# jackvial/tuatara

Measured on AMD Instinct MI355X. Metric: pages/sec whole-node (1024x768, ~40 crops/page), higher is better.
Workload: dtype f16x4

## Files before the change

### tuatara_amd/csrc/capi_debug.cpp

```cpp
#include "engine.h"

using namespace ttr;

extern "C" {

int ttr_dbg_conv(ttr_engine* e, const float* in0, int C0, const float* in1, int C1, int relu0, int relu1, int B, int H, int W, int ks, int dil,
                 const float* wgt, const float* bias, int Cout, int act, float* out) {
  TTR_GUARD_BEGIN
  Engine& E = *e->e;
  EngineScope lk(E);
  const size_t M = (size_t)B * H * W;
  const int K = ks * ks * (C0 + C1);
  DevBuf d0, d1, dout;
  Linear L;
  auto up = [&](DevBuf& d, const float* src, size_t nel) {
    d.ensure(nel * E.es);
    if (E.prec == kBF16) {
      std::vector<uint16_t> hbuf(nel);
      for (size_t i = 0; i < nel; ++i) hbuf[i] = f32_to_bf16_rne(src[i]);
      TTR_HIP_CHECK(hipMemcpy(d.p, hbuf.data(), nel * 2, hipMemcpyHostToDevice));
    } else TTR_HIP_CHECK(hipMemcpy(d.p, src, nel * 4, hipMemcpyHostToDevice));
  };
  up(d0, in0, M * C0);
  if (C1) up(d1, in1, M * C1);
// ... 308 lines not shown

void ttr_set_gemm_config(int cfg) { set_gemm_config(cfg); }

void ttr_set_decoder_mode(int mode) { g_tuning_default.decoder_mode = mode; }

void ttr_last_host_us(ttr_engine* e, float out[8]) { for (int i = 0; i < 8; ++i) out[i] = e ? e->e->host_us[i] : 0.f; }

int ttr_dbg_dec_stamps_ext(unsigned long long* out, int n) { return g_dec_dbg && n >= 0 && n <= 4096 && hipMemcpy(out, g_dec_dbg, (size_t)n * 8, hipMemcpyDeviceToHost) == hipSuccess ? 0 : -1; }
int ttr_dbg_dec_stamps(unsigned long long* out) { return g_dec_dbg && hipMemcpy(out, g_dec_dbg, 26 * 16 * 8, hipMemcpyDeviceToHost) == hipSuccess ? 0 : -1; }

int ttr_set_tuning(const char* key, int value) {
  const std::string k = key ? key : "";
  if (g_tuning_default.set(k, value)) return 0;
  if (k == "gemm_config") set_gemm_config(value);
  else if (k == "self_refine") set_dec_self_refine(value);
  else if (k == "cross_mfma") set_dec_cross_mfma(value);
  else if (k == "cross_crop") set_dec_cross_crop(value);
  else if (k == "cross_split") set_dec_cross_split(value);
  else if (k == "cross_rows_hsplit") set_dec_cross_rows_hsplit(value);
  else if (k == "mlp_store_nt") set_mlp_store_nt(value);
  else if (k == "mlp_stagger") set_mlp_stagger(value);
  else if (k == "c3s_wgs") set_conv3s_wgs_per_cu(value);
  else if (k == "c3_c32") set_conv3p_c32_tile(value);
  else if (k == "c3_narrow64") set_conv3p_narrow_bn64(value);
  else if (k == "upsample_block") set_upsample_block(value);
  else if (k == "mlp_ablate") set_mlp_ablate(value);
  else if (k == "attn_impl") set_attn_impl(value);
  else if (k == "ws_dbg_flags") set_gemm_ws_dbg_flags(value);
  else if (k == "ws_lean") set_gemm_ws_lean(value);
  else if (k == "store_policy") set_store_policy(value);
  else if (k == "head_persistent") set_conv3p_head_persistent(value);
  else if (k == "up_resident") set_gemm2_up_resident(value);
  else if (k == "up_2d") set_gemm2_up_2d(value);
  else if (k == "c3h_wgs_per_cu") set_conv3h_wgs_per_cu(value);
  else if (k == "g2_x_ring3") set_gemm2_x_ring3(value);
  else if (k == "g2_split_reuse") set_gemm2_split_reuse(value);
  else if (k == "g2_split_cfg") set_gemm2_split_cfg(value);
  else if (k == "g2_split_few") set_gemm2_split_few(value);
  else if (k == "g2_split_dbg") set_gemm2_split_dbg(value);
  else if (k == "g2_split_wreg") set_gemm2_split_wreg(value);
  else if (k == "g2_split_stream") set_gemm2_split_stream(value);
  else if (k == "g2_split_stream4") set_gemm2_split_stream4(value);
  else if (k == "gsp_sched") set_gemm_sp_sched(value);
  else if (k == "gsp_few") set_gemm_sp_few(value);
  else if (k == "gsp_epi") set_gemm_sp_epi(value);
  else if (k == "gsp_ks3") set_gemm_sp_ks3(value);
  else if (k == "gsp_stagger") set_gemm_sp_stagger(value);
  else if (k == "gsp_dbg") set_gemm_sp_dbg(value);
  else if (k == "gsp_stag") set_gemm_sp_stag(value);
  else if (k == "gsp_stagger_groups") set_gemm_sp_stagger_groups(value);
  else if (k == "qkv_attn_dbg") set_qkv_attn_dbg(value);
  else if (k == "qkv_attn4") set_qkv_attn4(value);
  else if (k == "skx_ln_max_rows") set_gemm_skx_ln_max_rows(value);
  else if (k == "c3_xs1_max_cin") set_conv3p_single_stage_max_cin(value);
  else if (k == "c3_force_bn128") set_conv3p_force_bn128(value);
  else if (k == "c3_c64_waves") set_conv3p_c64_waves(value);
  else if (k == "c3_c128_waves") set_conv3p_c128_waves(value);
  else if (k == "c3_narrow_wide") set_conv3p_narrow_wide(value);
  else if (k == "c3_narrow_frac") set_conv3p_narrow_frac(value);
  else if (k == "c3_narrowest_frac") set_conv3p_narrowest_frac(value);
  else if (k == "c3_deep_w") set_conv3p_deep_w(value);
  else if (k == "c3_deep_w64") set_conv3p_deep_w64(value);
  else if (k == "c3_first_persistent") set_conv3p_first_persistent(value);
  else if (k == "sk_max_rows") set_skinny_max_rows(value);
  else if (k == "ws_min_rows") set_gemm_ws_min_rows(value);
  else if (k == "dec_stamps") {
    if (value && !g_dec_dbg) { void* d = nullptr; if (hipMalloc(&d, 4096 * 8) != hipSuccess) return -1; (void)hipMemset(d, 0, 4096 * 8); g_dec_dbg = (unsigned long long*)d; }
    if (!value) g_dec_dbg = nullptr;
    set_gemm_ws_stamps(value == 2 ? g_dec_dbg : nullptr);
    set_conv3p_stamps(value == 4 ? g_dec_dbg : nullptr);
    set_mlp_stamps(value == 3 ? g_dec_dbg : nullptr);
    set_qkv_attn_stamps(value == 5 ? g_dec_dbg : nullptr);
    set_qkv_attn4_stamps(value == 5 ? g_dec_dbg : nullptr);
    set_conv3h_stamps(value == 6 ? g_dec_dbg : nullptr);
  }
  else return -1;
  return 0;
}

int ttr_engine_set_tuning(ttr_engine* e, const char* key, int value) {
  TTR_GUARD_BEGIN
  if (!e) return -1;
  const std::string k = key ? key : "";
  {
    std::lock_guard<std::mutex> lk(e->e->mu);
    if (e->e->tn.set(k, value)) return 0;
  }
  return ttr_set_tuning(key, value);
  TTR_GUARD_END(-1)
}

int ttr_bench_conv(ttr_engine* e, int B, int H, int W, int C0, int C1, int ks, int dil, int Cout, int act, int f32_resid, int iters, float* avg_us) {
  TTR_GUARD_BEGIN
  Engine& E = *e->e;
  EngineScope lk(E);
  const size_t M = (size_t)B * H * W;
  const int K = ks * ks * (C0 + C1);
  DevBuf d0, d1, dw, db, dout, dres;
  d0.ensure(M * C0 * E.es); launch_fill_random(E.prec, d0.p, M * C0, 1u, 1.0f, E.stream);
  if (C1) { d1.ensure(M * C1 * E.es); launch_fill_random(E.prec, d1.p, M * C1, 2u, 1.0f, E.stream); }
  dw.ensure((size_t)Cout * K * E.es); launch_fill_random(E.prec, dw.p, (size_t)Cout * K, 3u, 1.0f / std::sqrt((float)K), E.stream);
  db.ensure((size_t)Cout * 4); launch_fill_random(kF32, db.p, Cout, 4u, 1.0f, E.stream);
  ConvParams p{};
  p.in0 = d0.p; p.C0 = C0; p.in1 = C1 ? d1.p : nullptr; p.C1 = C1;
  p.B = B; p.H = H; p.W = W; p.ks = ks; p.dil = dil; p.wgt = dw.p; p.bias = db.as<float>();
  p.Cout = Cout; p.M = (int)M; p.act = act;
// ... 95 lines not shown
```

### tuatara_amd/csrc/engine.h

```cpp
#pragma once
#include <algorithm>
#include <cmath>
#include <cstdio>
#include <cstring>
#include <fstream>
#include <iostream>
#include <iterator>
#include <map>
#include <memory>
#include <mutex>
#include <chrono>
#include <dlfcn.h>
#include <arpa/inet.h>
#include <netdb.h>
#include <netinet/in.h>
#include <netinet/tcp.h>
#include <sys/socket.h>
#include <unistd.h>
#include <rccl/rccl.h>

#include <atomic>
#include <functional>
#include <condition_variable>
#include <thread>
#include <stdexcept>
#include <string>
#include <vector>

#include "../../include/tuatara_hip_debug.h"
#include "common.h"
#include "geometry.h"
#include "host_util.h"
#include "kernels.h"

namespace ttr {


extern thread_local std::string g_last_error;
extern unsigned long long* g_dec_dbg;
struct Tuning {
  int dbg_bf16_out = 0;
  int qkv_attn = 1;
  int qkv_attn_min = 160;
  int mlp_proj = 1;
  int mlp_min_rows = 49152;
  int dec_mlp_fused = 1;
  int dec_mlp_min_rows = 16384;
  int mlp_fused = 1;
  int tok_fuse = 1;
  int ln_fuse = 1;
  int fuse_first = 1;
  int qkv_attn_split = 1;
  int skinny_split = 1;
  int skinny_max_rows = 2048;
  int skx_ln_fuse = 1;
  int embed_fold = 1;
  int argmax_fold = 1;
  int sp_tiled_x = 1;
  int sp_tiled_w = 1;
  int ar_host_check = 10;
  int enc_chunk = 0;
  int enc_ln_pairs = 1;
  int dec_planes = 1;
  int qkv_kv_pairs = 1;
  int enc_fc2_pairs = 1;
  int craft_products = 3;
  int gpu_calipers = 1;
  int up_commute = 1;
  int head_tail = 1;
  int first_fused = 1;
  int head_packed = 1;
  int detector_only = 0;
  int bench_grid_boxes = 0;
  int split_planes = 1;
  int split_conv3p = 1;
  int split_gemm = 1;
  int craft_group = 16;
  int ar_tail_step = 12;
  int ar_crop_exit = 1;
  int ar_early_exit = 1;
  int decoder_mode = 1;
  int sp_hidden16 = 0;
  int craft_lanes = 1;
  int recog_overlap = 1;
  int images_batch = 32;
  int range_guard = 1;
  bool set(const std::string& k, int value) {
    if (k == "decoder_mode") decoder_mode = value;
    else if (k == "enc_chunk") enc_chunk = value;
    else if (k == "range_guard") range_guard = value;
    else if (k == "recog_overlap") recog_overlap = value;
    else if (k == "craft_lanes") craft_lanes = value == 2 ? 2 : 1;
    else if (k == "sp_hidden16") sp_hidden16 = value;
    else if (k == "images_batch") images_batch = value < 1 ? 1 : (value > 256 ? 256 : value);
    else if (k == "up_commute") up_commute = value;
    else if (k == "gpu_calipers") gpu_calipers = value;
    else if (k == "skinny_split") skinny_split = value;
    else if (k == "skinny_max_rows") skinny_max_rows = value;
    else if (k == "ar_host_check") ar_host_check = value;
    else if (k == "sp_tiled_w") sp_tiled_w = value;
    else if (k == "sp_tiled_x") sp_tiled_x = value;
    else if (k == "argmax_fold") argmax_fold = value;
    else if (k == "embed_fold") embed_fold = value;
    else if (k == "skx_ln_fuse") skx_ln_fuse = value;
    else if (k == "qkv_attn_split") qkv_attn_split = value;
    else if (k == "fuse_first") fuse_first = value;
    else if (k == "ln_fuse") ln_fuse = value;
// ... 560 lines not shown
```

### tuatara_amd/csrc/engine_parseq.cpp

```cpp
#include "engine.h"

namespace ttr {

unsigned long long* g_dec_dbg = nullptr;

void Engine::sgemm(const Linear& L, const void* in_planes, int M, void* out, int out_ld, int act, int out_planes,
           float* out_f32, int out_f32_ld, const float* resid, int resid_ld, int np, int resid_mod, int out_full_cols,
           const char* kind, int x_tiled, int out_tiled) {
  if (!L.ws.p) throw std::runtime_error("split GEMM: the layer has no weight planes");
  range_tag("parseq." + range_scope + (kind ? kind : "linear"));
  ConvParams p{};
  p.out_full_cols = out_full_cols;
  p.in0 = in_planes; p.C0 = L.k; p.B = 1; p.H = 1; p.W = M; p.ks = 1; p.dil = 1;
  p.wgt = L.ws.p; p.bias = L.b.as<float>(); p.split = np; p.out_scale = L.inv_scale; p.out_planes = out_planes == 1 ? 3 : out_planes;
  p.wgt_tiled = tn.sp_tiled_w ? L.wst.p : nullptr;
  p.x_tiled = x_tiled; p.out_tiled = out_tiled;
  p.store_policy = out_tiled == 2 && tn.sp_hidden16 == 2 ? 1 : 0;
  p.out = out; p.out_ld = out_ld; p.out_f32 = out_f32; p.out_f32_ld = out_f32_ld; p.resid = resid; p.resid_ld = resid_ld; p.resid_mod = resid_mod;
  p.Cout = L.cout_valid ? L.cout_valid : L.cout; p.M = M; p.act = act;
  p.skip = cur_skip; p.skip_n = cur_skip_n;
  const bool skinny = tn.skinny_split && np == 4 && M <= tn.skinny_max_rows && !x_tiled && !out_tiled && gemm_skx_eligible(p);
  if (!skinny) { if (const char* e = gemm2_check(p)) throw std::runtime_error(e); }
  if (skinny) {
    timed(kind ? kind : "split linear (triples, skinny)", 2.0 * M * p.Cout * L.k, 2.0 * M * p.Cout * L.k * np, [&] { launch_gemm_skx(p, stream); });
// ... 53 lines not shown
    p.Cout = L.cout_valid ? L.cout_valid : L.cout; p.M = rows; p.act = act;
    p.skip = cur_skip; p.skip_n = cur_skip_n;
    if (tn.skx_ln_fuse && tn.skinny_split && L.ws.p && gemm_skx_ln_eligible(p)) {
      timed(kind, 2.0 * rows * p.Cout * L.k, 2.0 * rows * p.Cout * L.k * 4, [&] { launch_gemm_skx(p, stream); });
      return;
    }
    lnp(nm, pa);
    sgemm(L, pa, rows, out, out_ld, act, out_planes, out_f32, out_f32_ld, nullptr, 0, 4, 0, 0, kind);
  };
  range_tag("parseq.decoder.self_attn.out_proj");
  sgemm(pq.at("self_out"), sa, rows, nullptr, 0, kActNone, 0, tgt, 384, resid_pos, 384, 4, resid_mod);
  ln_lin(d + "norm1", pq.at("cross_q"), q384, 384, kActNone, 0, nullptr, 0, "dec.norm1 + cross_q");
  range_tag("parseq.decoder.cross_attn");
  launch_dec_cross_attn(kF32, q384, kvmem, pb, N, R, stream, cur_skip, cur_skip_n, done_tok, done_col, 3);
  sgemm(pq.at("cross_out"), pb, rows, nullptr, 0, kActNone, 0, tgt, 384, tgt, 384);
  ln_lin(d + "norm2", pq.at("ffn1"), p1536, 1536, kActGelu, 3, nullptr, 0, "dec.norm2 + ffn1");
  sgemm(pq.at("ffn2"), p1536, rows, nullptr, 0, kActNone, 0, tgt, 384, tgt, 384);
  const Linear& head = pq.at("head");
  if (head.ws.p && tn.skinny_split && rows <= tn.skinny_max_rows)
    ln_lin("decoder.norm", head, nullptr, 0, kActNone, 0, logits_out, logits_ld, "dec.norm + head (skinny)");
  else ln_gemm(tgt, "decoder.norm", 1e-5f, t384, head, rows, nullptr, 0, kActNone, logits_out, logits_ld);
}

void Engine::decoder_tail(const void* sa, int N, int R, const float* resid_pos, int resid_mod, float* tgt, void* t384, void* t384b, void* t1536,
                  const void* kvmem, float* logits_out, int logits_ld, const int* done_tok, int done_col) {
  const int rows = N * R;
  const std::string d = "decoder.layers.0.";
  gemm(pq.at("self_out"), sa, rows, nullptr, 0, kActNone, tgt, 384, resid_pos, 384, resid_mod);
  ln_gemm(tgt, d + "norm1", 1e-5f, t384, pq.at("cross_q"), rows, t384b, 384, kActNone);
  launch_dec_cross_attn(prec, t384b, kvmem, t384, N, R, stream, cur_skip, cur_skip_n, done_tok, done_col);
  const int dec_panels = (rows + 127) / 128, dec_cus = device_cu_count(256), dec_rounds = (dec_panels + dec_cus - 1) / dec_cus;
  const bool dec_fill = tn.dec_mlp_fused == 2 || dec_panels * 100 >= 65 * dec_rounds * dec_cus;
  if (R > 1 && prec == kBF16 && gemm_config() >= 0 && tn.dec_mlp_fused && rows >= tn.dec_mlp_min_rows && dec_fill) {
    MlpParams q{};
    q.x = tgt; q.x_out = tgt; q.M = rows;
    q.ln_g = pqf.at(d + "norm2.weight").as<float>(); q.ln_b = pqf.at(d + "norm2.bias").as<float>(); q.ln_eps = 1e-5f;
    q.w1p = dec_ffn1_packed.as<bf16>(); q.b1 = pq.at("ffn1").b.as<float>();
    q.w2p = dec_ffn2_packed.as<bf16>(); q.b2 = pq.at("ffn2").b.as<float>();
    q.nln_g = pqf.at("decoder.norm.weight").as<float>(); q.nln_b = pqf.at("decoder.norm.bias").as<float>(); q.nln_eps = 1e-5f; q.nln_out = (bf16*)t384b;
    q.att = (const bf16*)t384; q.wpp = dec_co_packed.as<bf16>(); q.bp = pq.at("cross_out").b.as<float>();
    timed("mlp_fused (refinement block)", 2.0 * rows * 384 * 1536 * 2 + 2.0 * rows * 384 * 384, 2.0 * rows * 384 * 1536 * 2 + 2.0 * rows * 384 * 384, [&] { launch_mlp_fused(q, stream); });
    gemm(pq.at("head"), t384b, rows, nullptr, 0, kActNone, logits_out, logits_ld);
    return;
  }
  gemm(pq.at("cross_out"), t384, rows, nullptr, 0, kActNone, tgt, 384, tgt, 384, 0);
  ln_gemm(tgt, d + "norm2", 1e-5f, t384, pq.at("ffn1"), rows, t1536, 1536, kActGelu);
  gemm(pq.at("ffn2"), t1536, rows, nullptr, 0, kActNone, tgt, 384, tgt, 384, 0);
  ln_gemm(tgt, "decoder.norm", 1e-5f, t384, pq.at("head"), rows, nullptr, 0, kActNone, logits_out, logits_ld);
}

void Engine::parseq_forward(const uint8_t* d_crops, int N, float* d_logits, float* d_ar, int* d_ids, float* d_prob, float* d_conf, const RowMask* row_masks,
                            int* d_alt_ids, float* d_alt_prob) {
  if (N <= 0) return;
  constexpr int kMaxCrops = 4096;
  if (N > kMaxCrops) {
    const int groups = (N + kMaxCrops - 1) / kMaxCrops, per = (N + groups - 1) / groups;
    for (int g0 = 0; g0 < N; g0 += per) {
      const int n = std::min(per, N - g0);
      parseq_forward(d_crops + (size_t)g0 * 32 * 128 * 3, n, d_logits + (size_t)g0 * 26 * 95, d_ar ? d_ar + (size_t)g0 * 26 * 95 : nullptr, d_ids + (size_t)g0 * 26,
                     d_prob + (size_t)g0 * 26, d_conf + g0, row_masks ? row_masks + g0 : nullptr,
                     d_alt_ids ? d_alt_ids + (size_t)g0 * 26 * alts : nullptr, d_alt_prob ? d_alt_prob + (size_t)g0 * 26 * alts : nullptr);
    }
    return;
  }
  if ((charset.restricts() || row_masks) && prec == kBF16) throw std::runtime_error("parseq_forward: a character set needs an f16x4 or f32 engine (the bf16 engine's kernels take no class mask)");
  prof_stage = 1;
  const int M = N * 128, E = 384;
  const int patch_ld = pq.at("patch").k;
  range_tag("parseq.encoder.patch_embed");
  void* patches = (pq_ws[0].ensure((size_t)M * patch_ld * es), pq_ws[0].p);
  float* x = (float*)(pq_ws[1].ensure((size_t)M * E * 4), pq_ws[1].p);
  void* t384 = (pq_ws[2].ensure((size_t)std::max(M, N * 26) * E * es), pq_ws[2].p);
  void* tbig = (pq_ws[3].ensure((size_t)M * 1536 * es), pq_ws[3].p);
  void* att = (pq_ws[4].ensure((size_t)std::max(M, N * 26) * E * es), pq_ws[4].p);
  launch_patchify(prec, d_crops, patches, N, patch_ld, stream);
  gemm(pq.at("patch"), patches, M, nullptr, 0, kActNone, x, E, pqf.at("encoder.pos_embed").as<float>(), E, 128);
  const bool enc_split = prec == kSplit && tn.split_gemm && tn.split_planes;
  if (enc_split) {
    int CHS = std::max(1, std::min(N, (int)((((size_t)1 << 31) - 1) / ((size_t)128 * 1536 * 6))));
    if (tn.enc_chunk > 0) CHS = std::min(CHS, tn.enc_chunk);
    if (N > CHS) { const int groups = (N + CHS - 1) / CHS; CHS = (N + groups - 1) / groups; }
    void* lnp = (pq_ws[11].ensure((size_t)M * E * 6), pq_ws[11].p);
    void* bigp = (pq_ws[12].ensure((size_t)std::min(N, CHS) * 128 * 1536 * 6), pq_ws[12].p);
    void* attp = (pq_ws[13].ensure((size_t)std::min(N, CHS) * 128 * E * 6), pq_ws[13].p);
    auto lnp_at = [&](int c0) { return (char*)lnp + (size_t)c0 * 128 * E * 6; };
    const int lnpl = tn.enc_ln_pairs ? 2 : 3;
    const int xt = tn.sp_tiled_x && tn.qkv_attn_split && lnpl == 2 && tn.enc_fc2_pairs && std::min(CHS, N) * 128 > tn.skinny_max_rows ? 1 : 0;
    for (int c0 = 0; c0 < N; c0 += CHS) {
      const int nc = std::min(CHS, N - c0), Mc = nc * 128;
      float* xc = x + (size_t)c0 * 128 * E;
      for (int l = 0; l < 12; ++l) {
        const std::string p = "encoder.blocks." + std::to_string(l) + ".";
        range_scope = p;
        range_tag("parseq." + p + "norm1");
        launch_layernorm_planes(xc, E, pqf.at(p + "norm1.weight").as<float>(), pqf.at(p + "norm1.bias").as<float>(), 1e-6f, lnp_at(c0), Mc, stream, lnpl, nullptr, 0, xt);
        if (tn.qkv_attn_split && lnpl == 2) {
          const Linear& L = pq.at(p + "qkv_hm");
          range_tag("parseq." + p + "attn (qkv + attention)");
          const double qa = 2.0 * Mc * 3 * E * E, aa = 2.0 * 2 * nc * 6 * 128.0 * 128 * 64;
          timed("enc.qkv+attention: gemm_sp_kernel<128,192,NP=3,EPI=1>", qa + aa, qa * 3 + aa * 3.5,
                [&] { launch_qkv_attn_split(lnp_at(c0), L.ws.p, L.b.as<float>(), L.inv_scale, attp, nc, stream, tn.sp_tiled_w ? L.wst.p : nullptr, xt, xt); });
        } else {
        sgemm(pq.at(p + "qkv"), lnp_at(c0), Mc, bigp, 3 * E, kActNone, 1, nullptr, 0, nullptr, 0, lnpl + 1, 0, tn.qkv_kv_pairs ? E : 0, "enc.qkv");
        range_tag("parseq." + p + "attn.qkv"), launch_attn_enc_split(bigp, attp, nc, stream);
        }
        sgemm(pq.at(p + "proj"), attp, Mc, nullptr, 0, kActNone, 0, xc, E, xc, E, 4, 0, 0, "enc.proj", xt, 0);
        range_tag("parseq." + p + "norm2");
// ... 209 lines not shown
```

### tuatara_amd/csrc/gemm_skx.hip

```cpp
#include <stdexcept>

#include "common.h"
#include "kernels.h"
#include "split.h"

namespace ttr {

namespace {
__device__ __forceinline__ __amdgpu_buffer_rsrc_t skx_rsrc(const void* base, unsigned bytes) {
  return __builtin_amdgcn_make_buffer_rsrc(const_cast<void*>(base), 0, (int)bytes, 0x00020000);
}
__device__ __forceinline__ f16x8 skx_load(__amdgpu_buffer_rsrc_t rs, unsigned voff, unsigned soff) {
  return __builtin_bit_cast(f16x8, __builtin_amdgcn_raw_buffer_load_b128(rs, voff, soff, 0));
}
constexpr int SKX_BN = 32, SKX_DEPTH = 3;
}

template <int RB, bool LNP = false, bool ROWM = false>
__global__ __launch_bounds__(256) void gemm_skx_kernel(ConvParams p) {
  static_assert(!LNP || RB == 1, "the LayerNorm prologue is the 16-row form's");
  static_assert(!ROWM || LNP, "row masks belong to the token prologue");
  __shared__ __attribute__((aligned(16))) float part[4][2][RB][64][4];
  __shared__ int skip_now;
  if (p.skip) {
    if (LNP && p.done_count) {
      if (threadIdx.x == 0) skip_now = __builtin_nontemporal_load(p.skip) >= p.skip_n;
      __syncthreads();
      if (skip_now) return;
    } else if (__builtin_nontemporal_load(p.skip) >= p.skip_n) return;
  }
  constexpr int XROW = 3 * 384 + 8;
  __shared__ __attribute__((aligned(16))) f16 xs[LNP ? 16 * XROW : 8];
  const int tid = threadIdx.x, lane = tid & 63;
  const int wave = __builtin_amdgcn_readfirstlane(tid >> 6);
  const int q = lane & 15, g = lane >> 4;
  RangeWatch rw;
  const int K = p.C0, nsteps = K >> 5;
  const int n0 = blockIdx.x * SKX_BN, m0 = blockIdx.y * (16 * RB);
  const __amdgpu_buffer_rsrc_t rsx = skx_rsrc(p.in0, (unsigned)((size_t)p.M * K * 6));
  const __amdgpu_buffer_rsrc_t rsw = skx_rsrc(p.wgt, (unsigned)((size_t)p.Cout * K * 6));
  constexpr unsigned OOB = 0x80000000u;
  unsigned xo[RB], wo[2];
#pragma unroll
  for (int rb = 0; rb < RB; ++rb) { const int m = m0 + rb * 16 + q; xo[rb] = m < p.M ? ((unsigned)m * (unsigned)(3 * K) + g * 8) * 2u : OOB; }
#pragma unroll
  for (int cb = 0; cb < 2; ++cb) { const int n = n0 + cb * 16 + q; wo[cb] = n < p.Cout ? ((unsigned)n * (unsigned)(3 * K) + g * 8) * 2u : OOB; }

  struct Frags { f16x8 x[RB][3], w[2][2]; };
  auto fetch = [&](Frags& f, int step) {
    const unsigned ks = (unsigned)step * 64u;
    const unsigned dead = step < nsteps ? 0u : OOB;
    if constexpr (!LNP) {
#pragma unroll
      for (int rb = 0; rb < RB; ++rb)
#pragma unroll
        for (int pl = 0; pl < 3; ++pl) f.x[rb][pl] = skx_load(rsx, xo[rb] | dead, ks + (unsigned)(pl * K) * 2u);
    }
#pragma unroll
    for (int cb = 0; cb < 2; ++cb) {
      f.w[cb][0] = skx_load(rsw, wo[cb] | dead, ks);
      f.w[cb][1] = skx_load(rsw, wo[cb] | dead, ks + (unsigned)(2 * K) * 2u);
    }
  };
  f32x4 acc[2][RB];
#pragma unroll
  for (int cb = 0; cb < 2; ++cb)
#pragma unroll
    for (int rb = 0; rb < RB; ++rb) acc[cb][rb] = f32x4{0.f, 0.f, 0.f, 0.f};
  const f16 dn = (f16)(1.f / 2048.f);
  const f16x8 dnv = {dn, dn, dn, dn, dn, dn, dn, dn};
  auto multiply = [&](const Frags& f) {
#pragma unroll
    for (int cb = 0; cb < 2; ++cb) {
      const f16x8 w0b = f.w[cb][0] * dnv;
#pragma unroll
      for (int rb = 0; rb < RB; ++rb) {
        f32x4 a = acc[cb][rb];
        a = __builtin_amdgcn_mfma_f32_16x16x32_f16(f.w[cb][0], f.x[rb][0], a, 0, 0, 0);
        a = __builtin_amdgcn_mfma_f32_16x16x32_f16(w0b, f.x[rb][1], a, 0, 0, 0);
        a = __builtin_amdgcn_mfma_f32_16x16x32_f16(w0b, f.x[rb][2], a, 0, 0, 0);
        acc[cb][rb] = __builtin_amdgcn_mfma_f32_16x16x32_f16(f.w[cb][1], f.x[rb][0], a, 0, 0, 0);
      }
    }
  };
  Frags fb[SKX_DEPTH];
  const int mine = (nsteps - wave + 3) >> 2;
  const int rounds = (mine + SKX_DEPTH - 1) / SKX_DEPTH;
#pragma unroll
  for (int d = 0; d < SKX_DEPTH; ++d) { fetch(fb[d], wave + 4 * d); __builtin_amdgcn_sched_barrier(0); }
  if constexpr (LNP) {
    constexpr int D = 384;
    const bool act = lane < 48;
    const int c = (act ? lane : 0) * 8;
    int mrow[4]; bool live[4];
#pragma unroll
    for (int rr = 0; rr < 4; ++rr) { mrow[rr] = m0 + wave + 4 * rr; live[rr] = mrow[rr] < p.M; }
    float v[4][8];
    if (p.tok) {
      int token[4] = {0, 0, 0, 0};
      if (p.tok_logits) {
        float best[4]; int bi[4];
        if (p.tok_C <= 128) {
          float t0[4], t1[4];
          const bool ok0 = lane < p.tok_C && p.tok_mask.allows(lane), ok1 = lane + 64 < p.tok_C && p.tok_mask.allows(lane + 64);
          bool rok0[4], rok1[4];
          if constexpr (ROWM) {
#pragma unroll
            for (int rr = 0; rr < 4; ++rr) {
              const RowClassMask rm = row_class_mask(p.tok_mask, p.tok_row_masks, live[rr] ? mrow[rr] : m0);
              rok0[rr] = lane < p.tok_C && rm.allows(lane); rok1[rr] = lane + 64 < p.tok_C && rm.allows(lane + 64);
            }
          }
#pragma unroll
          for (int rr = 0; rr < 4; ++rr) {
            const float* lg = p.tok_logits + (int64_t)(live[rr] ? mrow[rr] : m0) * p.tok_logits_ld;
            t0[rr] = lane < p.tok_C ? lg[lane] : -INFINITY;
            t1[rr] = lane + 64 < p.tok_C ? lg[lane + 64] : -INFINITY;
          }
#pragma unroll
          for (int rr = 0; rr < 4; ++rr) {
            best[rr] = -INFINITY; bi[rr] = 0x7fffffff;
            const bool k0 = ROWM ? rok0[rr] : ok0, k1 = ROWM ? rok1[rr] : ok1;
            if (k0 && t0[rr] > best[rr]) { best[rr] = t0[rr]; bi[rr] = lane; }
            if (k1 && t1[rr] > best[rr]) { best[rr] = t1[rr]; bi[rr] = lane + 64; }
          }
        } else {
#pragma unroll
          for (int rr = 0; rr < 4; ++rr) {
            const float* lg = p.tok_logits + (int64_t)(live[rr] ? mrow[rr] : m0) * p.tok_logits_ld;
            best[rr] = -INFINITY; bi[rr] = 0x7fffffff;
            if constexpr (ROWM) {
              const RowClassMask rm = row_class_mask(p.tok_mask, p.tok_row_masks, live[rr] ? mrow[rr] : m0);
              for (int cc = lane; cc < p.tok_C; cc += 64) { const float t = lg[cc]; if (rm.allows(cc) && t > best[rr]) { best[rr] = t; bi[rr] = cc; } }
            } else
            for (int cc = lane; cc < p.tok_C; cc += 64) { const float t = lg[cc]; if (p.tok_mask.allows(cc) && t > best[rr]) { best[rr] = t; bi[rr] = cc; } }
          }
        }
#pragma unroll
        for (int rr = 0; rr < 4; ++rr) {
#pragma unroll
          for (int o = 32; o > 0; o >>= 1) {
            const float ov = __shfl_xor(best[rr], o); const int oi = __shfl_xor(bi[rr], o);
            if (ov > best[rr] || (ov == best[rr] && oi < bi[rr])) { best[rr] = ov; bi[rr] = oi; }
          }
          token[rr] = bi[rr];
        }
        if (blockIdx.x == 0 && lane == 0) {
#pragma unroll
          for (int rr = 0; rr < 4; ++rr) {
            if (!live[rr]) continue;
            const int m = mrow[rr];
            p.tok[m * p.tok_ld + p.tok_col] = bi[rr];
            if (p.done_count && bi[rr] == p.tok_eos) {
              bool first = true;
              for (int cc = 1; cc < p.tok_col; ++cc) first = first && p.tok[m * p.tok_ld + cc] != p.tok_eos;
              if (first) atomicAdd(p.done_count, 1);
            }
          }
        }
      } else {
#pragma unroll
        for (int rr = 0; rr < 4; ++rr) token[rr] = live[rr] ? p.tok[mrow[rr] * p.tok_ld + p.tok_col] : 0;
      }
      float4 pa = make_float4(0.f, 0.f, 0.f, 0.f), pb = pa;
      if (p.tok_pos) { pa = *reinterpret_cast<const float4*>(p.tok_pos + c); pb = *reinterpret_cast<const float4*>(p.tok_pos + c + 4); }
#pragma unroll
      for (int rr = 0; rr < 4; ++rr) {
        int tk = token[rr];
        tk = tk < 0 ? 0 : (tk > p.tok_max ? p.tok_max : tk);
        const float* x = p.tok_emb + (int64_t)tk * D + c;
        const float4 a = *reinterpret_cast<const float4*>(x), b = *reinterpret_cast<const float4*>(x + 4);
        v[rr][0] = a.x; v[rr][1] = a.y; v[rr][2] = a.z; v[rr][3] = a.w; v[rr][4] = b.x; v[rr][5] = b.y; v[rr][6] = b.z; v[rr][7] = b.w;
        if (p.tok_pos) {
          v[rr][0] = pa.x + v[rr][0]; v[rr][1] = pa.y + v[rr][1]; v[rr][2] = pa.z + v[rr][2]; v[rr][3] = pa.w + v[rr][3];
          v[rr][4] = pb.x + v[rr][4]; v[rr][5] = pb.y + v[rr][5]; v[rr][6] = pb.z + v[rr][6]; v[rr][7] = pb.w + v[rr][7];
        }
      }
    } else {
#pragma unroll
      for (int rr = 0; rr < 4; ++rr) {
        const float* x = p.ln_in + (int64_t)(live[rr] ? mrow[rr] : m0) * p.ln_ld + c;
        const float4 a = *reinterpret_cast<const float4*>(x), b = *reinterpret_cast<const float4*>(x + 4);
        v[rr][0] = a.x; v[rr][1] = a.y; v[rr][2] = a.z; v[rr][3] = a.w; v[rr][4] = b.x; v[rr][5] = b.y; v[rr][6] = b.z; v[rr][7] = b.w;
      }
    }
#pragma unroll
    for (int rr = 0; rr < 4; ++rr) {
      const int rl = wave + 4 * rr;
      f16x8 o0 = {0, 0, 0, 0, 0, 0, 0, 0}, o1 = o0, o2 = o0;
      if (live[rr]) {
        float y[8];
        ln384_row8(v[rr], act, p.ln_gamma + c, p.ln_beta + c, p.ln_eps, y);
        split3_x8(y, o0, o1, o2, rw);
      }
      if (act) {
        f16* d = xs + rl * XROW + c;
        *reinterpret_cast<f16x8*>(d) = o0; *reinterpret_cast<f16x8*>(d + D) = o1; *reinterpret_cast<f16x8*>(d + 2 * D) = o2;
      }
    }
    __syncthreads();
#pragma unroll
    for (int d = 0; d < SKX_DEPTH; ++d)
#pragma unroll
      for (int pl = 0; pl < 3; ++pl) fb[d].x[0][pl] = *reinterpret_cast<const f16x8*>(xs + q * XROW + pl * D + (wave + 4 * d) * 32 + g * 8);
  }
  for (int r = 0; r < rounds; ++r) {
#pragma unroll
    for (int d = 0; d < SKX_DEPTH; ++d) {
      multiply(fb[d]);
      __builtin_amdgcn_sched_barrier(0);
      fetch(fb[d], wave + 4 * ((r + 1) * SKX_DEPTH + d));
      __builtin_amdgcn_sched_barrier(0);
    }
  }
#pragma unroll
  for (int cb = 0; cb < 2; ++cb)
#pragma unroll
    for (int rb = 0; rb < RB; ++rb) *reinterpret_cast<f32x4*>(&part[wave][cb][rb][lane][0]) = acc[cb][rb];
  __syncthreads();
#pragma unroll
  for (int pr = 0; pr < 2 * RB; ++pr) {
    if ((pr & 3) != wave) continue;
    const int cb = pr / RB, rb = pr % RB;
    f32x4 v = *reinterpret_cast<const f32x4*>(&part[0][cb][rb][lane][0]);
#pragma unroll
    for (int w = 1; w < 4; ++w) v += *reinterpret_cast<const f32x4*>(&part[w][cb][rb][lane][0]);
    const int n = n0 + cb * 16 + 4 * g, m = m0 + rb * 16 + q;
    if (n >= p.Cout || m >= p.M) continue;
    float o[4];
    const bool vec = n + 3 < p.Cout;
    float bv[4] = {0.f, 0.f, 0.f, 0.f};
    if (p.bias) {
      if (vec) { const float4 b4 = *reinterpret_cast<const float4*>(p.bias + n); bv[0] = b4.x; bv[1] = b4.y; bv[2] = b4.z; bv[3] = b4.w; }
      else { for (int e = 0; e < 4; ++e) if (n + e < p.Cout) bv[e] = p.bias[n + e]; }
    }
#pragma unroll
    for (int e = 0; e < 4; ++e) o[e] = fmaf(v[e], p.out_scale, bv[e]);
    if (p.resid) {
      const float* rp = p.resid + (int64_t)(p.resid_mod ? m % p.resid_mod : m) * p.resid_ld + n;
      if (vec && ((p.resid_ld & 3) | ((uintptr_t)p.resid & 15)) == 0) { const float4 r = *reinterpret_cast<const float4*>(rp); o[0] += r.x; o[1] += r.y; o[2] += r.z; o[3] += r.w; }
      else { for (int e = 0; e < 4; ++e) if (n + e < p.Cout) o[e] += rp[e]; }
    }
    if (p.act == kActRelu) {
#pragma unroll
      for (int e = 0; e < 4; ++e) o[e] = fmaxf(o[e], 0.f);
    } else if (p.act == kActGelu) {
#pragma unroll
      for (int e = 0; e < 4; ++e) o[e] = gelu_exact(o[e]);
    }
    if (p.out) {
      if (p.out_planes == 3) {
        f16x2 a0, b0, c0, a1, b1, c1;
        split3_pair(o[0], o[1], a0, b0, c0, rw); split3_pair(o[2], o[3], a1, b1, c1, rw);
        typedef __attribute__((ext_vector_type(4))) _Float16 f16x4;
        f16* d = reinterpret_cast<f16*>(p.out) + (int64_t)m * (3 * (int64_t)p.out_ld) + n;
        *reinterpret_cast<f16x4*>(d) = f16x4{a0[0], a0[1], a1[0], a1[1]};
        *reinterpret_cast<f16x4*>(d + p.out_ld) = f16x4{b0[0], b0[1], b1[0], b1[1]};
        *reinterpret_cast<f16x4*>(d + 2 * p.out_ld) = f16x4{c0[0], c0[1], c1[0], c1[1]};
      } else if (p.out_planes == 2) {
        f16x2 a0, b0, a1, b1;
        split2_pair(o[0], o[1], a0, b0, rw); split2_pair(o[2], o[3], a1, b1, rw);
        typedef __attribute__((ext_vector_type(4))) _Float16 f16x4;
        f16* d = reinterpret_cast<f16*>(p.out) + (int64_t)m * (2 * (int64_t)p.out_ld) + n;
        *reinterpret_cast<f16x4*>(d) = f16x4{a0[0], a0[1], a1[0], a1[1]};
        *reinterpret_cast<f16x4*>(d + p.out_ld) = f16x4{b0[0], b0[1], b1[0], b1[1]};
      } else {
        float* d = reinterpret_cast<float*>(p.out) + (int64_t)m * p.out_ld + n;
        if (vec && ((p.out_ld & 3) | ((uintptr_t)p.out & 15)) == 0) *reinterpret_cast<float4*>(d) = make_float4(o[0], o[1], o[2], o[3]);
        else { for (int e = 0; e < 4; ++e) if (n + e < p.Cout) d[e] = o[e]; }
      }
    }
    if (p.out_f32) {
      float* d = p.out_f32 + (int64_t)m * p.out_f32_ld + n;
      if (vec && ((p.out_f32_ld & 3) | ((uintptr_t)p.out_f32 & 15)) == 0) *reinterpret_cast<float4*>(d) = make_float4(o[0], o[1], o[2], o[3]);
      else { for (int e = 0; e < 4; ++e) if (n + e < p.Cout) d[e] = o[e]; }
    }
  }
  rw.flush(p.range_flag, p.range_tag);
}

static int g_skx_ln_max_rows = 2048;
void set_gemm_skx_ln_max_rows(int v) { g_skx_ln_max_rows = v; }
bool gemm_skx_ln_eligible(const ConvParams& p) {
  if ((!p.ln_in && !p.tok) || !p.ln_gamma || !p.ln_beta || p.C0 != 384 || p.M > (p.tok ? 256 : g_skx_ln_max_rows)) return false;
  if (p.tok ? (!p.tok_emb || (((uintptr_t)p.tok_emb | (uintptr_t)p.tok_pos) & 15)) : (p.ln_ld % 4 != 0 || ((uintptr_t)p.ln_in & 15))) return false;
  if (((uintptr_t)p.ln_gamma | (uintptr_t)p.ln_beta) & 15) return false;
  ConvParams q = p;
  q.in0 = p.wgt;
  return gemm_skx_eligible(q);
}

bool gemm_skx_eligible(const ConvParams& p) {
  if (p.split != 4 || p.ks != 1 || p.C1 != 0 || p.out_pool || p.out_relu || p.M <= 0 || p.Cout <= 0 || p.C0 % 32 != 0 || p.out_full_cols) return false;
  if ((size_t)p.M * p.C0 * 6 >= ((size_t)1 << 31) || (p.M + 63) / 64 > 65535) return false;
  if ((size_t)((p.Cout + 7) / 8 * 8) * p.C0 * 6 >= ((size_t)1 << 31)) return false;
  if (p.out && p.out_planes && (p.Cout % 4 || p.out_ld % 4 || ((uintptr_t)p.out & 15))) return false;
  if (((uintptr_t)p.out | (uintptr_t)p.out_f32 | (uintptr_t)p.resid) & 3) return false;
  return !(((uintptr_t)p.in0 | (uintptr_t)p.wgt | (uintptr_t)p.bias) & 15);
}

void launch_gemm_skx(const ConvParams& p_in, hipStream_t s) {
  const ConvParams p = with_range_ctx(p_in);
  if (p.ln_in || p.tok) {
    if (!gemm_skx_ln_eligible(p)) throw std::runtime_error("gemm_skx: LayerNorm prologue: shape not supported");
    const dim3 grid((p.Cout + SKX_BN - 1) / SKX_BN, (p.M + 15) / 16);
    if (p.tok_row_masks && p.tok_logits) hipLaunchKernelGGL((gemm_skx_kernel<1, true, true>), grid, dim3(256), 0, s, p);
    else hipLaunchKernelGGL((gemm_skx_kernel<1, true>), grid, dim3(256), 0, s, p);
    return;
  }
  if (!gemm_skx_eligible(p)) throw std::runtime_error("gemm_skx: shape not supported");
  const int rbsel = p.M <= 256 ? 1 : 4;
  const dim3 grid((p.Cout + SKX_BN - 1) / SKX_BN, (p.M + 16 * rbsel - 1) / (16 * rbsel)), block(256);
  if (rbsel == 1) hipLaunchKernelGGL(gemm_skx_kernel<1>, grid, block, 0, s, p);
  else hipLaunchKernelGGL(gemm_skx_kernel<4>, grid, block, 0, s, p);
}

}
```

### tuatara_amd/csrc/kernels.h

```cpp
#pragma once
#include <stdexcept>
#include "common.h"

namespace ttr {

struct RangeCtx { unsigned* flag = nullptr; unsigned tag = 0; };
RangeCtx& range_ctx();
inline ConvParams with_range_ctx(const ConvParams& p) {
  ConvParams q = p;
  if (!q.range_flag) { q.range_flag = range_ctx().flag; q.range_tag = range_ctx().tag; }
  return q;
}

unsigned* tile_counters(hipStream_t s);

const char* igemm_check(const ConvParams& p);
void launch_igemm(Precision prec, const ConvParams& p, hipStream_t s);
void set_gemm_config(int cfg);
int gemm_config();

const char* gemm2_check(const ConvParams& p);
void launch_gemm2(const ConvParams& p, int cfg, hipStream_t s);
void set_gemm2_split_dbg(int v);
void set_gemm2_split_wreg(int v);
void set_gemm2_split_stream(int v);
void set_gemm2_split_stream4(int v);
bool gemm_sp_eligible(const ConvParams& p);
void set_gemm_sp_sched(int v);
void set_gemm_sp_few(int v);
void set_gemm_sp_epi(int v);
void set_gemm_sp_ks3(int v);
void set_gemm_sp_dbg(int v);
void set_gemm_sp_stag(int v);
void set_gemm_sp_stagger(int v);
void set_gemm_sp_stagger_groups(int v);
void set_qkv_attn_dbg(int v);
void set_qkv_attn_stamps(unsigned long long* dev_buf);
bool gemm_sp_ks3_eligible(const ConvParams& p);
void launch_gemm_sp_ks3(const ConvParams& p, int cfg, hipStream_t s);
void set_gemm_skx_ln_max_rows(int v);
void launch_gemm_sp(const ConvParams& p, int cfg, hipStream_t s);
void set_gemm2_split_cfg(int v);
void set_gemm2_split_few(int v);
void set_gemm2_split_reuse(int v);
void set_gemm2_x_ring3(int v);
const void* gelu_lut_for_current_device();
const void* gelu_hermite_lut_for_current_device();
bool gemm_skx_eligible(const ConvParams& p);
bool gemm_skx_ln_eligible(const ConvParams& p);
void launch_gemm_skx(const ConvParams& p, hipStream_t s);
const char* gemm_sk_check(const ConvParams& p);
void launch_gemm_sk(const ConvParams& p, hipStream_t s);
void set_skinny_max_rows(int m);
void set_mlp_store_nt(int v);
void set_mlp_stamps(unsigned long long* dev_buf);
void launch_dec_cross_attn_mfma(const bf16* q, const bf16* kvmem, bf16* out, int N, int R, hipStream_t s);
void launch_dec_cross_attn_split(const float* q, const float* kvmem, void* out_planes, int N, int R, hipStream_t s);
void set_dec_cross_rows_hsplit(int v);
void set_dec_cross_split(int v);
void set_dec_cross_crop(int v);
void set_dec_cross_mfma(int v);
void set_dec_self_refine(int v);
void set_conv3p_stamps(unsigned long long* dev_buf);
void set_gemm_ws_stamps(unsigned long long* dev_buf);
extern int g_store_policy;
void set_store_policy(int v);
bool conv1u_eligible(const ConvParams& p);
void launch_conv1u(const ConvParams& p, hipStream_t s);
void set_qkv_attn4(int v);
int qkv_attn4_enabled();
void set_qkv_attn4_stamps(unsigned long long* dev_buf);
void launch_qkv_attn4(const void* x_pairs, const void* w_planes, const float* bias, float inv_scale, void* out_planes, int N, hipStream_t s, const void* w_tiled, int x_tiled,
                      int out_tiled);
void set_gemm2_up_resident(int v);
void set_gemm2_up_2d(int v);
bool conv3h_eligible(const ConvParams& p);
void launch_conv3h(const ConvParams& p, hipStream_t s);
void set_conv3h_wgs_per_cu(int v);
void set_conv3h_stamps(unsigned long long* dev_buf);
void set_conv3p_head_persistent(int v);
void set_gemm_ws_dbg_flags(int f);
void set_gemm_ws_lean(int v);
int skinny_max_rows();
const char* gemm_ws_check(const ConvParams& p);
void launch_gemm_ws(const ConvParams& p, hipStream_t s);
void set_gemm_ws_min_rows(int m);
struct Conv3sParams {
  const bf16* in;
  const bf16* wgt;
  const float* bias;
  bf16* out;
  const bf16* w6; const float* b6;
  const bf16* w8; const float* b8;
  float* heat;
  int B, H, W;
};
const char* conv3s_check(const Conv3sParams& p);
void launch_conv3s(const Conv3sParams& p, hipStream_t s);
void set_conv3s_wgs_per_cu(int v);
const char* conv3p_check(const ConvParams& p);
void launch_conv3p(const ConvParams& p, hipStream_t s);
int conv3p_split_bn(const ConvParams& p);
// ... 131 lines not shown
```

Before: 420.8.

## Add 64-row LayerNorm-prologue skinny GEMM and two-workgroup occupancy variant

Extends the LayerNorm-prologue skinny GEMM to 64-row workgroups (RB=4), staging four 16-row LN blocks with prefetch of the next block's rows. Row counts above 256 now use the wider workgroups, which reuses each weight tile across more rows. Adds a launch-bounds variant that asks for two workgroups per CU for the 64-row forms. It also raises the skinny-path row limits from 2048 to kMaxCrops (4096), so more GEMMs take this path. The trade-offs are extra register pressure from the double-buffered rows and the risk of spilling under the tighter launch bound.

```diff
diff --git a/tuatara_amd/csrc/capi_debug.cpp b/tuatara_amd/csrc/capi_debug.cpp
--- a/tuatara_amd/csrc/capi_debug.cpp
+++ b/tuatara_amd/csrc/capi_debug.cpp
@@ -384,6 +384,8 @@
   else if (k == "qkv_attn_dbg") set_qkv_attn_dbg(value);
   else if (k == "qkv_attn4") set_qkv_attn4(value);
   else if (k == "skx_ln_max_rows") set_gemm_skx_ln_max_rows(value);
+  else if (k == "skx_ln_rb1_max_rows") set_gemm_skx_ln_rb1_max_rows(value);
+  else if (k == "skx_w2") set_gemm_skx_w2(value);
   else if (k == "c3_xs1_max_cin") set_conv3p_single_stage_max_cin(value);
   else if (k == "c3_force_bn128") set_conv3p_force_bn128(value);
   else if (k == "c3_c64_waves") set_conv3p_c64_waves(value);
diff --git a/tuatara_amd/csrc/engine.h b/tuatara_amd/csrc/engine.h
--- a/tuatara_amd/csrc/engine.h
+++ b/tuatara_amd/csrc/engine.h
@@ -52,7 +52,7 @@
   int fuse_first = 1;
   int qkv_attn_split = 1;
   int skinny_split = 1;
-  int skinny_max_rows = 2048;
+  int skinny_max_rows = kMaxCrops;
   int skx_ln_fuse = 1;
   int embed_fold = 1;
   int argmax_fold = 1;
diff --git a/tuatara_amd/csrc/engine_parseq.cpp b/tuatara_amd/csrc/engine_parseq.cpp
--- a/tuatara_amd/csrc/engine_parseq.cpp
+++ b/tuatara_amd/csrc/engine_parseq.cpp
@@ -129,7 +129,6 @@
 void Engine::parseq_forward(const uint8_t* d_crops, int N, float* d_logits, float* d_ar, int* d_ids, float* d_prob, float* d_conf, const RowMask* row_masks,
                             int* d_alt_ids, float* d_alt_prob) {
   if (N <= 0) return;
-  constexpr int kMaxCrops = 4096;
   if (N > kMaxCrops) {
     const int groups = (N + kMaxCrops - 1) / kMaxCrops, per = (N + groups - 1) / groups;
     for (int g0 = 0; g0 < N; g0 += per) {
diff --git a/tuatara_amd/csrc/gemm_skx.hip b/tuatara_amd/csrc/gemm_skx.hip
--- a/tuatara_amd/csrc/gemm_skx.hip
+++ b/tuatara_amd/csrc/gemm_skx.hip
@@ -16,10 +16,11 @@
 constexpr int SKX_BN = 32, SKX_DEPTH = 3;
 }
 
-template <int RB, bool LNP = false, bool ROWM = false>
-__global__ __launch_bounds__(256) void gemm_skx_kernel(ConvParams p) {
-  static_assert(!LNP || RB == 1, "the LayerNorm prologue is the 16-row form's");
-  static_assert(!ROWM || LNP, "row masks belong to the token prologue");
+template <int RB, bool LNP = false, bool ROWM = false, bool W2 = false>
+__global__ __launch_bounds__(256, W2 ? 2 : 1) void gemm_skx_kernel(ConvParams p) {
+  static_assert(!W2 || RB == 4, "the 16-row forms fit several workgroups per CU as they are");
+  static_assert(!LNP || RB == 1 || RB == 4, "the LayerNorm prologue: 16-row or 64-row workgroups");
+  static_assert(!ROWM || (LNP && RB == 1), "row masks belong to the token prologue (16-row workgroups)");
   __shared__ __attribute__((aligned(16))) float part[4][2][RB][64][4];
   __shared__ int skip_now;
   if (p.skip) {
@@ -95,8 +96,18 @@
     int mrow[4]; bool live[4];
 #pragma unroll
     for (int rr = 0; rr < 4; ++rr) { mrow[rr] = m0 + wave + 4 * rr; live[rr] = mrow[rr] < p.M; }
-    float v[4][8];
-    if (p.tok) {
+    float vb[RB > 1 ? 2 : 1][4][8];
+    auto& v = vb[0];
+    auto load_rows = [&](int rb, float (&t)[4][8]) {
+#pragma unroll
+      for (int rr = 0; rr < 4; ++rr) {
+        const int m = m0 + rb * 16 + wave + 4 * rr;
+        const float* x = p.ln_in + (int64_t)(m < p.M ? m : m0) * p.ln_ld + c;
+        const float4 a = *reinterpret_cast<const float4*>(x), b = *reinterpret_cast<const float4*>(x + 4);
+        t[rr][0] = a.x; t[rr][1] = a.y; t[rr][2] = a.z; t[rr][3] = a.w; t[rr][4] = b.x; t[rr][5] = b.y; t[rr][6] = b.z; t[rr][7] = b.w;
+      }
+    };
+    if (RB == 1 && p.tok) {
       int token[4] = {0, 0, 0, 0};
       if (p.tok_logits) {
         float best[4]; int bi[4];
@@ -176,33 +187,39 @@
           v[rr][4] = pb.x + v[rr][4]; v[rr][5] = pb.y + v[rr][5]; v[rr][6] = pb.z + v[rr][6]; v[rr][7] = pb.w + v[rr][7];
         }
       }
-    } else {
+    } else load_rows(0, v);
+#pragma unroll
+    for (int rb = 0; rb < RB; ++rb) {
+      if (rb > 0 && m0 + rb * 16 >= p.M) {
+#pragma unroll
+        for (int d = 0; d < SKX_DEPTH; ++d)
+#pragma unroll
+          for (int pl = 0; pl < 3; ++pl) fb[d].x[rb][pl] = f16x8{0, 0, 0, 0, 0, 0, 0, 0};
+        continue;
+      }
+      float (&vr)[4][8] = vb[rb & (RB > 1 ? 1 : 0)];
+      if (rb + 1 < RB) load_rows(rb + 1, vb[(rb + 1) & (RB > 1 ? 1 : 0)]);
 #pragma unroll
       for (int rr = 0; rr < 4; ++rr) {
-        const float* x = p.ln_in + (int64_t)(live[rr] ? mrow[rr] : m0) * p.ln_ld + c;
-        const float4 a = *reinterpret_cast<const float4*>(x), b = *reinterpret_cast<const float4*>(x + 4);
-        v[rr][0] = a.x; v[rr][1] = a.y; v[rr][2] = a.z; v[rr][3] = a.w; v[rr][4] = b.x; v[rr][5] = b.y; v[rr][6] = b.z; v[rr][7] = b.w;
-      }
-    }
-#pragma unroll
-    for (int rr = 0; rr < 4; ++rr) {
-      const int rl = wave + 4 * rr;
-      f16x8 o0 = {0, 0, 0, 0, 0, 0, 0, 0}, o1 = o0, o2 = o0;
-      if (live[rr]) {
-        float y[8];
-        ln384_row8(v[rr], act, p.ln_gamma + c, p.ln_beta + c, p.ln_eps, y);
-        split3_x8(y, o0, o1, o2, rw);
-      }
-      if (act) {
-        f16* d = xs + rl * XROW + c;
-        *reinterpret_cast<f16x8*>(d) = o0; *reinterpret_cast<f16x8*>(d + D) = o1; *reinterpret_cast<f16x8*>(d + 2 * D) = o2;
-      }
-    }
-    __syncthreads();
-#pragma unroll
-    for (int d = 0; d < SKX_DEPTH; ++d)
-#pragma unroll
-      for (int pl = 0; pl < 3; ++pl) fb[d].x[0][pl] = *reinterpret_cast<const f16x8*>(xs + q * XROW + pl * D + (wave + 4 * d) * 32 + g * 8);
+        const int rl = wave + 4 * rr;
+        f16x8 o0 = {0, 0, 0, 0, 0, 0, 0, 0}, o1 = o0, o2 = o0;
+        if (m0 + rb * 16 + rl < p.M) {
+          float y[8];
+          ln384_row8(vr[rr], act, p.ln_gamma + c, p.ln_beta + c, p.ln_eps, y);
+          split3_x8(y, o0, o1, o2, rw);
+        }
+        if (act) {
+          f16* d = xs + rl * XROW + c;
+          *reinterpret_cast<f16x8*>(d) = o0; *reinterpret_cast<f16x8*>(d + D) = o1; *reinterpret_cast<f16x8*>(d + 2 * D) = o2;
+        }
+      }
+      __syncthreads();
+#pragma unroll
+      for (int d = 0; d < SKX_DEPTH; ++d)
+#pragma unroll
+        for (int pl = 0; pl < 3; ++pl) fb[d].x[rb][pl] = *reinterpret_cast<const f16x8*>(xs + q * XROW + pl * D + (wave + 4 * d) * 32 + g * 8);
+      if (rb + 1 < RB && m0 + (rb + 1) * 16 < p.M) __syncthreads();
+    }
   }
   for (int r = 0; r < rounds; ++r) {
 #pragma unroll
@@ -279,8 +296,12 @@
   rw.flush(p.range_flag, p.range_tag);
 }
 
-static int g_skx_ln_max_rows = 2048;
+static int g_skx_ln_max_rows = kMaxCrops;
+static int g_skx_ln_rb1_max_rows = 256;
 void set_gemm_skx_ln_max_rows(int v) { g_skx_ln_max_rows = v; }
+void set_gemm_skx_ln_rb1_max_rows(int v) { g_skx_ln_rb1_max_rows = v; }
+static int g_skx_w2 = 1;
+void set_gemm_skx_w2(int v) { g_skx_w2 = v; }
 bool gemm_skx_ln_eligible(const ConvParams& p) {
   if ((!p.ln_in && !p.tok) || !p.ln_gamma || !p.ln_beta || p.C0 != 384 || p.M > (p.tok ? 256 : g_skx_ln_max_rows)) return false;
   if (p.tok ? (!p.tok_emb || (((uintptr_t)p.tok_emb | (uintptr_t)p.tok_pos) & 15)) : (p.ln_ld % 4 != 0 || ((uintptr_t)p.ln_in & 15))) return false;
@@ -303,8 +324,11 @@
   const ConvParams p = with_range_ctx(p_in);
   if (p.ln_in || p.tok) {
     if (!gemm_skx_ln_eligible(p)) throw std::runtime_error("gemm_skx: LayerNorm prologue: shape not supported");
-    const dim3 grid((p.Cout + SKX_BN - 1) / SKX_BN, (p.M + 15) / 16);
-    if (p.tok_row_masks && p.tok_logits) hipLaunchKernelGGL((gemm_skx_kernel<1, true, true>), grid, dim3(256), 0, s, p);
+    const int rows = !p.tok && p.M > g_skx_ln_rb1_max_rows ? 64 : 16;
+    const dim3 grid((p.Cout + SKX_BN - 1) / SKX_BN, (p.M + rows - 1) / rows);
+    if (rows == 64 && g_skx_w2) hipLaunchKernelGGL((gemm_skx_kernel<4, true, false, true>), grid, dim3(256), 0, s, p);
+    else if (rows == 64) hipLaunchKernelGGL((gemm_skx_kernel<4, true>), grid, dim3(256), 0, s, p);
+    else if (p.tok_row_masks && p.tok_logits) hipLaunchKernelGGL((gemm_skx_kernel<1, true, true>), grid, dim3(256), 0, s, p);
     else hipLaunchKernelGGL((gemm_skx_kernel<1, true>), grid, dim3(256), 0, s, p);
     return;
   }
@@ -312,6 +336,7 @@
   const int rbsel = p.M <= 256 ? 1 : 4;
   const dim3 grid((p.Cout + SKX_BN - 1) / SKX_BN, (p.M + 16 * rbsel - 1) / (16 * rbsel)), block(256);
   if (rbsel == 1) hipLaunchKernelGGL(gemm_skx_kernel<1>, grid, block, 0, s, p);
+  else if (g_skx_w2) hipLaunchKernelGGL((gemm_skx_kernel<4, false, false, true>), grid, block, 0, s, p);
   else hipLaunchKernelGGL(gemm_skx_kernel<4>, grid, block, 0, s, p);
 }
 
diff --git a/tuatara_amd/csrc/kernels.h b/tuatara_amd/csrc/kernels.h
--- a/tuatara_amd/csrc/kernels.h
+++ b/tuatara_amd/csrc/kernels.h
@@ -38,7 +38,6 @@
 void set_qkv_attn_stamps(unsigned long long* dev_buf);
 bool gemm_sp_ks3_eligible(const ConvParams& p);
 void launch_gemm_sp_ks3(const ConvParams& p, int cfg, hipStream_t s);
-void set_gemm_skx_ln_max_rows(int v);
 void launch_gemm_sp(const ConvParams& p, int cfg, hipStream_t s);
 void set_gemm2_split_cfg(int v);
 void set_gemm2_split_few(int v);
@@ -46,8 +45,12 @@
 void set_gemm2_x_ring3(int v);
 const void* gelu_lut_for_current_device();
 const void* gelu_hermite_lut_for_current_device();
+constexpr int kMaxCrops = 4096;
 bool gemm_skx_eligible(const ConvParams& p);
 bool gemm_skx_ln_eligible(const ConvParams& p);
+void set_gemm_skx_ln_max_rows(int v);
+void set_gemm_skx_w2(int v);
+void set_gemm_skx_ln_rb1_max_rows(int v);
 void launch_gemm_skx(const ConvParams& p, hipStream_t s);
 const char* gemm_sk_check(const ConvParams& p);
 void launch_gemm_sk(const ConvParams& p, hipStream_t s);
```

Result: no change. 418.3 (-0.6%).
